# LouisBearing/BirdSoundClassif

Hardware: AMD Instinct MI355X
Metric: clips/sec (3 s @ 22.05 kHz) detect fwd (higher is better)
Workload: dtype f32; 1 GPU; BASELINE.json configs[1]: 1xMI355X inference, batch=64 synthetic 3 s clips (PCM16 @22.05 kHz resident in HBM) through the HIP STFT front end + detector forward + device post-processing, detections returned to the host; batch_per_gpu=64, distinct_clips=64, lanes=2

## Files before the change

birdsoundclassif_amd/_lib.py:

```python
import ctypes as C
import os
import subprocess

_HERE = os.path.dirname(os.path.abspath(__file__))
LIB_PATH = os.environ.get('NBM_LIB') or os.path.join(_HERE, 'libnbm_hip.so')
CSRC = os.path.join(_HERE, 'csrc')

_lib = None


class GemmDesc(C.Structure):
    _fields_ = [('x', C.c_void_p), ('w', C.c_void_p), ('y', C.c_void_p),
                ('scale', C.c_void_p), ('shift', C.c_void_p), ('residual', C.c_void_p),
                ('x_gs', C.c_int64), ('w_gs', C.c_int64), ('y_gs', C.c_int64), ('res_gs', C.c_int64),
                ('groups', C.c_int),
                ('B', C.c_int), ('H', C.c_int), ('W', C.c_int), ('Cin', C.c_int),
                ('N', C.c_int),
                ('kh', C.c_int), ('kw', C.c_int), ('stride', C.c_int), ('pad', C.c_int),
                ('Ho', C.c_int), ('Wo', C.c_int),
                ('x_ld', C.c_int), ('w_ld', C.c_int), ('y_ld', C.c_int), ('res_ld', C.c_int),
                ('alpha', C.c_float), ('act', C.c_int), ('shift_per_row', C.c_int),
                ('up', C.c_void_p), ('up_H', C.c_int), ('up_W', C.c_int),
                ('rows', C.c_void_p), ('rows_blocks', C.c_void_p),
                ('rows_mode', C.c_int), ('rows_count', C.c_int), ('rows_TH', C.c_int), ('rows_TW', C.c_int),
# ... 42 lines not shown
                ('B', C.c_int), ('H', C.c_int), ('W', C.c_int), ('Cin', C.c_int), ('N', C.c_int),
                ('kh', C.c_int), ('kw', C.c_int), ('stride', C.c_int), ('pad', C.c_int), ('Ho', C.c_int), ('Wo', C.c_int),
                ('g_ld', C.c_int), ('w_ld', C.c_int), ('x_ld', C.c_int), ('out_ld', C.c_int), ('res_ld', C.c_int),
                ('mask_ld', C.c_int), ('alpha', C.c_float), ('bias_grad', C.c_void_p), ('residual2', C.c_void_p), ('res2_ld', C.c_int),
                ('mask_bits', C.c_void_p)]


class GemmPlan(C.Structure):
    _fields_ = [('name', C.c_char_p), ('rc', C.c_int), ('kernel', C.c_int), ('grid', C.c_int * 3), ('block', C.c_int),
                ('m_tiles', C.c_int), ('n_tiles', C.c_int), ('vec_epi', C.c_int), ('fast', C.c_int), ('slices', C.c_int),
                ('phased', C.c_int), ('ph_tiles', C.c_int * 4), ('splits', C.c_int), ('k_chunk', C.c_int),
                ('plain', C.c_int), ('b_generic', C.c_int), ('narrow_m', C.c_int), ('halves', C.c_int)]


_P, _I, _L, _F, _U64, _U32 = C.c_void_p, C.c_int, C.c_int64, C.c_float, C.c_uint64, C.c_uint32

SIGNATURES = {
    'nbm_graph_census': [_P, C.POINTER(C.c_longlong * 6)],
    'nbm_copy_rect': [_P, _P, _L, _L, _I, _L, _L, _I, _I, _P],
    'nbm_gemm_conv': [C.POINTER(GemmDesc), _P],
    'nbm_gconv3x3': [C.POINTER(GconvDesc), _P],
    'nbm_gconv3x3_dgrad': [C.POINTER(GconvBwdDesc), _P],
    'nbm_gconv3x3_wgrad': [C.POINTER(GconvBwdDesc), _P],
    'nbm_gconv3x3_wgrad_workspace': [C.POINTER(GconvBwdDesc), C.POINTER(C.c_longlong)],
    'nbm_pcm16_to_wave': [_P, _L, _I, _I, _I, _P, _L, _L, _P, _L, _I, _I, _P],
    'nbm_resample_to_wave': [_P, _L, _I, _L, _I, _I, _P, _I, _L, _L, _P, _L, _I, _I, _I, _P],
    'nbm_wav_decode': [_P, _L, _I, _I, _I, _I, _L, _P, _L, _P],
    'nbm_minmax_init': [_P, _I, _P],
    'nbm_stft_db': [_P, _L, _I, _I, _I, _I, _P, _I, _I, _I, _F, _P, _L, _I, _P, _P],
    'nbm_spec_windows': [_P, _L, _I, _I, _I, _I, _P, _P, _I, _I, _I, _P, _P],
    'nbm_spec_windows_table': [_P, _I, _I, _P, _I, _I, _P],
    'nbm_init_conv': [_P, _L, _P, _P, _I, _P, _P],
    'nbm_stem7x7': [_P, _I, _I, _I, _P, _P, _P, _P, _P, _P, _P],
    'nbm_stem7x7_wgrad': [_P, _P, _I, _I, _I, _P, _P, _P],
    'nbm_maxpool3x3s2': [_P, _I, _I, _I, _I, _P, _I, _I, _P, _P],
    'nbm_space_to_batch2': [_P, _I, _I, _I, _I, _P, _I, _P],
    'nbm_avgpool2x2': [_P, _I, _I, _I, _I, _P, _P],
    'nbm_avgpool2x2_bwd': [_P, _I, _I, _I, _I, _P, _P],
    'nbm_upsample_bilinear_add': [_P, _I, _I, _I, _I, _P, _P, _I, _I, _P],
    'nbm_softmax_rows': [_P, _L, _I, _L, _P],
    'nbm_dwconv3x3': [_P, _I, _I, _I, _I, _I, _I, _P, _P, _P, _L, _P, _I, _I, _P],
    'nbm_dwconv_bn_act': [_P, _I, _I, _I, _I, _I, _I, _P, _P, _P, _I, _P, _I, _I, _P, _P],
    'nbm_dwconv_pool_slots': [_I, _I, _I],
    'nbm_dwconv_strip_rows': [],
    'nbm_se_gate': [_P, _I, _I, _I, _F, _P, _P, _I, _P, _P, _P, _P, _I, _I, _P, _I, _P],
    'nbm_silu': [_P, _P, _L, _P],
    'nbm_layernorm': [_P, _L, _I, _P, _P, _F, _P, _P],
    'nbm_mha_small': [_P, _P, _P, _I, _I, _I, _P, _I, _I, _I, _I, _I, _L, _L, _P, _F, _P],
    'nbm_mha_segments': [_P, _P, _P, _I, _I, _I, _P, _I, _I, _I, _I, _I, _I, _P, _P, _I, _F, _P],
    'nbm_pair_softmax': [_P, _L, _I, _I, _P, _I, _P],
    'nbm_rpn_decode': [_P, _P, _P, _I, _I, _I, _I, _I, _I, _P, _P, _P, _P],
    'nbm_nan_images': [_P, _I, _L, _P, _P],
    'nbm_rpn_select': [_P, _P, _P, _I, _I, _I, _I, _I, _P, _P, _P, _P, _P],
    'nbm_nms_batched': [_P, _P, _P, _I, _I, _F, _I, _P, _P, _P, _P, _P, _P, _P],
    'nbm_rpn_select_big_workspace': [_I, _I, C.POINTER(C.c_int64)],
    'nbm_rpn_select_big': [_P, _P, _P, _I, _I, _I, _I, _I, _P, _L, _P, _P, _P, _P, _P],
    'nbm_nms_big_workspace': [_I, _I, C.POINTER(C.c_int64)],
    'nbm_nms_big': [_P, _P, _P, _I, _I, _F, _I, _P, _L, _P, _P, _P, _P, _P],
    'nbm_roi_pool': [C.POINTER(RoiDesc), _P],
    'nbm_roi_pool_hw': [C.POINTER(RoiHwDesc), _P],
    'nbm_rcnn_post': [_P, _P, _I, _I, _P, _P, _I, _I, _I, _F, _F, _I, _P, _P, _P],
    'nbm_merge_collect': [_P, _P, _I, _I, _I, _I, _I, _L, _P, _P, _P, _P, _P, _P],
    'nbm_merge_nms_workspace': [_I, C.POINTER(C.c_int64)],
    'nbm_merge_nms': [_P, _P, _I, _F, _P, _L, _P, _P, _P],
    'nbm_merge_gather': [_P, _P, _P, _P, _P, _I, _P, _P, _P],
    'nbm_conv_dgrad': [C.POINTER(BwdDesc), _P],
# ... 113 lines not shown
```

birdsoundclassif_amd/csrc/stem.hip:

```cpp
#include "nbm_common.h"

namespace {

constexpr int SP = 264;
constexpr int KR = 8;
constexpr int KK = 7 * KR;
constexpr int OP = 68;
static_assert(7 * SP + KK * 64 <= 128 * OP, "operands must fit the output tile");

struct StemParams {
  const float* img; const float* weff; const float* wb; const float* wb_full; const float* scale; const float* shift;
  float* y;
  int B, H, W, Ho, Wo;
};

__global__ __launch_bounds__(256) void stem7x7_kernel(const StemParams p) {
  __shared__ __attribute__((aligned(16))) float smem[128 * OP];
  float* img_s = smem;
  float* w_s = smem + 7 * SP;
  __shared__ float cb_s[64 * 8];
  const int tid = threadIdx.x, lane = tid & 63, wave = tid >> 6;
  const int ox0 = blockIdx.x * 128, oy = blockIdx.y, b = blockIdx.z;

  const int ix0 = 2 * ox0 - 3;
  constexpr int NST = (7 * SP + 255) / 256;
  float stv[NST];
#pragma unroll
  for (int k = 0; k < NST; ++k) {
    const int i = min(tid + 256 * k, 7 * SP - 1);
    const int r = i / SP, c = i - r * SP;
    const int iy = min(max(2 * oy - 3 + r, 0), p.H - 1), ix = min(max(ix0 + c, 0), p.W - 1);
    stv[k] = p.img[((long long)b * p.H + iy) * p.W + ix];
  }
#pragma unroll
  for (int k = 0; k < NST; ++k) {
    const int i = tid + 256 * k;
    const int r = i / SP, c = i - r * SP;
    const int iy = 2 * oy - 3 + r, ix = ix0 + c;
    if (i < 7 * SP) img_s[i] = ((unsigned)iy < (unsigned)p.H && (unsigned)ix < (unsigned)p.W && c < 261) ? stv[k] : 0.f;
  }
  for (int i = tid; i < KK * 64 / 4; i += 256)
    reinterpret_cast<f32x4*>(w_s)[i] = reinterpret_cast<const f32x4*>(p.weff)[i];
  unsigned rmask = 0;
#pragma unroll
  for (int r = 0; r < 7; ++r)
    if ((unsigned)(2 * oy - 3 + r) < (unsigned)p.H) rmask |= 1u << r;
  const bool row_border = rmask != 0x7fu;
  const bool col_border = ox0 < 2 || 2 * (ox0 + 127) + 3 >= p.W;
  if (row_border || col_border)
    for (int i = tid; i < 64 * 7; i += 256) {
      const int n = i / 7, sx = i - n * 7;
      float a = 0.f;
      for (int r = 0; r < 7; ++r)
        if ((rmask >> r) & 1u) a += p.wb[n * 49 + r * 7 + sx];
      cb_s[n * 8 + sx] = a;
    }
  __syncthreads();

  const int pl = lane & 31, slot = lane >> 5;
  const float* a_base = img_s + 2 * (wave * 32 + pl) + slot;
  const float* b_base = w_s + slot * 64 + pl;
  f32x16 acc0, acc1;
#pragma unroll
  for (int e = 0; e < 16; ++e) { acc0[e] = 0.f; acc1[e] = 0.f; }
#pragma unroll
  for (int j = 0; j < KK / 2; ++j) {
    constexpr int dummy = 0; (void)dummy;
    const int r = (2 * j) / KR, s0 = (2 * j) % KR;
    const float a = a_base[r * SP + s0];
    const float b0 = b_base[(2 * j) * 64], b1 = b_base[(2 * j) * 64 + 32];
    acc0 = __builtin_amdgcn_mfma_f32_32x32x2f32(a, b0, acc0, 0, 0, 0);
    acc1 = __builtin_amdgcn_mfma_f32_32x32x2f32(a, b1, acc1, 0, 0, 0);
  }

  __syncthreads();
#pragma unroll
  for (int t = 0; t < 2; ++t) {
    const int n = 32 * t + pl;
    const float sc = p.scale[n], sh = p.shift[n];
    float bfull = p.wb_full[n];
    if (row_border) {
      bfull = 0.f;
#pragma unroll
      for (int s = 0; s < 7; ++s) bfull += cb_s[n * 8 + s];
    }
    const f32x16& acc = t == 0 ? acc0 : acc1;
#pragma unroll
    for (int e = 0; e < 16; ++e) {
      const int px = wave * 32 + (e & 3) + 8 * (e >> 2) + 4 * slot;
      const int ox = ox0 + px;
      float bias = bfull;
      if (col_border && (ox < 2 || 2 * ox + 3 >= p.W)) {
        bias = 0.f;
#pragma unroll
        for (int s = 0; s < 7; ++s)
          if ((unsigned)(2 * ox - 3 + s) < (unsigned)p.W) bias += cb_s[n * 8 + s];
      }
      smem[px * OP + n] = fmaxf((acc[e] + bias) * sc + sh, 0.f);
    }
  }
  __syncthreads();
  float* yrow = p.y + (((long long)b * p.Ho + oy) * p.Wo + ox0) * 64;
#pragma unroll
  for (int it = 0; it < 8; ++it) {
    const int px = it * 16 + (tid >> 4), c4 = (tid & 15) * 4;
    if (ox0 + px < p.Wo)
      *reinterpret_cast<f32x4*>(yrow + px * 64 + c4) = *reinterpret_cast<const f32x4*>(smem + px * OP + c4);
  }
}

struct StemWgradParams {
  const float* img; const float* g; float* D;
  int B, H, W, Ho, Wo, n_strips, tiles_x;
};

__global__ __launch_bounds__(256) void stem_wgrad_kernel(const StemWgradParams p) {
  __shared__ __attribute__((aligned(16))) float img_s[7 * SP];
  __shared__ __attribute__((aligned(16))) float g_s[128 * 64];
  const int tid = threadIdx.x, lane = tid & 63, wave = tid >> 6;
  const int mt = wave >> 1, nt = wave & 1;
  const int pl = lane & 31, slot = lane >> 5;
  const int col = nt * 32 + pl;
  const int r = col >> 3, sx = col & 7;
  const bool tap = col < 56 && sx < 7;
  const float ones = col == 56 ? 1.f : 0.f;
  const float* b_base = img_s + (tap ? r * SP + sx : 0) + 2 * slot;
  const float* a_base = g_s + slot * 64 + mt * 32 + pl;
  f32x16 acc;
#pragma unroll
  for (int e = 0; e < 16; ++e) acc[e] = 0.f;
  for (int strip = blockIdx.x; strip < p.n_strips; strip += gridDim.x) {
    const int tx = strip % p.tiles_x, rowi = strip / p.tiles_x;
    const int oy = rowi % p.Ho, b = rowi / p.Ho;
    const int ox0 = tx * 128, ix0 = 2 * ox0 - 3;
    __syncthreads();
    constexpr int NST = (7 * SP + 255) / 256;
    float stv[NST];
#pragma unroll
    for (int k = 0; k < NST; ++k) {
      const int i = min(tid + 256 * k, 7 * SP - 1);
// ... 83 lines not shown
extern "C" int nbm_stem7x7_wgrad(const float* img, const float* g, int B, int H, int W, float* D, float* Cb, void* stream) {
  if (!img || !g || !D || !Cb || B <= 0 || H <= 0 || W <= 0) return NBM_EINVAL;
  if (!nbm_aligned16(g)) return NBM_EALIGN;
  StemWgradParams p{};
  p.img = img; p.g = g; p.D = D; p.B = B; p.H = H; p.W = W;
  p.Ho = (H + 6 - 7) / 2 + 1; p.Wo = (W + 6 - 7) / 2 + 1;
  p.tiles_x = (p.Wo + 127) / 128;
  const long long strips = (long long)B * p.Ho * p.tiles_x;
  if (strips > 0x7fffffffll) return NBM_EUNSUPPORTED;
  p.n_strips = (int)strips;
  hipStream_t st = (hipStream_t)stream;
  if (nbm_zero_async(D, sizeof(float) * 64 * 64, st) != hipSuccess || nbm_zero_async(Cb, sizeof(float) * 64 * 49, st) != hipSuccess)
    return (int)hipGetLastError();
  const int grid = (int)(strips < 1024 ? strips : 1024);
  hipLaunchKernelGGL(stem_wgrad_kernel, dim3(grid), dim3(256), 0, st, p);
  int top = p.Ho < 2 ? p.Ho : 2, bot0 = top, left = p.Wo < 2 ? p.Wo : 2, right0 = left;
  while (bot0 < p.Ho && 2 * bot0 + 3 < H) ++bot0;
  while (right0 < p.Wo && 2 * right0 + 3 < W) ++right0;
  hipLaunchKernelGGL(stem_vborder_kernel, dim3(8, B), dim3(256), 0, st, g, H, W, p.Ho, p.Wo, top, bot0, left, right0, Cb);
  return nbm_launch_status();
}

extern "C" int nbm_stem7x7(const float* img, int B, int H, int W, const float* weff, const float* wb, const float* wb_full,
                           const float* scale, const float* shift, float* y, void* stream) {
  if (!img || !weff || !wb || !wb_full || !scale || !shift || !y || B <= 0 || H <= 0 || W <= 0) return NBM_EINVAL;
  if (!nbm_aligned16(weff)) return NBM_EALIGN;
  StemParams p{};
  p.img = img; p.weff = weff; p.wb = wb; p.wb_full = wb_full; p.scale = scale; p.shift = shift; p.y = y;
  p.B = B; p.H = H; p.W = W; p.Ho = (H + 6 - 7) / 2 + 1; p.Wo = (W + 6 - 7) / 2 + 1;
  dim3 grid((p.Wo + 127) / 128, p.Ho, B);
  hipLaunchKernelGGL(stem7x7_kernel, grid, dim3(256), 0, (hipStream_t)stream, p);
  return nbm_launch_status();
}
```

birdsoundclassif_amd/nets/backbone.py:

```python
import math

import torch
from torch import nn

from .. import ops
from . import _prep, functional as Fn
from .position_encoding import build_position_encoding

bcbk_channels = {'resnet': {'2': 64, '3': 256, '4': 512, '5': 1024, '6': 2048}}
_RESNET_LAYERS = {'resnet50': [3, 4, 6, 3], 'resnet101': [3, 4, 23, 3], 'resnet152': [3, 8, 36, 3]}
_RESNEXT = {'resnext50_32x4d': ([3, 4, 6, 3], 32, 4), 'resnext101_32x8d': ([3, 4, 23, 3], 32, 8),
            'resnext101_64x4d': ([3, 4, 23, 3], 64, 4)}
_EFFNET_BASE = ((1, 3, 1, 32, 16, 1), (6, 3, 2, 16, 24, 2), (6, 5, 2, 24, 40, 2), (6, 3, 2, 40, 80, 3), (6, 5, 1, 80, 112, 3),
                (6, 5, 2, 112, 192, 4), (6, 3, 1, 192, 320, 1))
_EFFICIENTNET = {'efficientnet_b0': (1.0, 1.0), 'efficientnet_b1': (1.0, 1.1), 'efficientnet_b2': (1.1, 1.2),
                 'efficientnet_b3': (1.2, 1.4), 'efficientnet_b4': (1.4, 1.8)}
_EFFNET_TAPS = (1, 2, 3, 5, 7)


def _make_divisible(v, divisor=8):
    new_v = max(divisor, int(v + divisor / 2) // divisor * divisor)
    return new_v + divisor if new_v < 0.9 * v else new_v


def efficientnet_stages(name):
    width, depth = _EFFICIENTNET[name]
    return [(t, k, s, _make_divisible(i * width), _make_divisible(o * width), int(math.ceil(n * depth))) for t, k, s, i, o, n in _EFFNET_BASE]


class FrozenBatchNorm2d(nn.Module):

    def __init__(self, n):
        super().__init__()
        self.register_buffer('weight', torch.ones(n))
        self.register_buffer('bias', torch.zeros(n))
        self.register_buffer('running_mean', torch.zeros(n))
        self.register_buffer('running_var', torch.ones(n))

    def _load_from_state_dict(self, state_dict, prefix, local_metadata, strict, missing_keys, unexpected_keys,
                              error_msgs):
        state_dict.pop(prefix + 'num_batches_tracked', None)
        super()._load_from_state_dict(state_dict, prefix, local_metadata, strict, missing_keys, unexpected_keys,
                                      error_msgs)

    def affine(self):
        return _prep.bn_affine(self.weight, self.bias, self.running_mean, self.running_var, 1e-5, frozen=True)


class BatchNorm2d(nn.BatchNorm2d):

# ... 121 lines not shown
            s, b = self.downsample[1].affine()
            idt = Fn.conv(x, self.downsample[0].weight, scale=s, shift=b, stride=self.stride)
        else:
            idt = x
        s, b = self.bn3.affine()
        return Fn.conv(o, self.conv3.weight, scale=s, shift=b, residual=idt, act=ops.ACT_RELU)


class _ResNetBody(nn.Module):

    def __init__(self, layers, norm_layer, dilation=False, groups=1, base_width=64):
        super().__init__()
        self.conv1 = nn.Conv2d(3, 64, 7, stride=2, padding=3, bias=False)
        self.bn1 = norm_layer(64)
        self.dilation = bool(dilation)
        inplanes = 64
        for li, (planes, n, stride) in enumerate(zip((64, 128, 256, 512), layers, (1, 2, 2, 1 if dilation else 2)), start=1):
            blocks = []
            for bi in range(n):
                st = stride if bi == 0 else 1
                ds = None
                if bi == 0 and (st != 1 or inplanes != planes * 4):
                    ds = nn.Sequential(nn.Conv2d(inplanes, planes * 4, 1, stride=st, bias=False), norm_layer(planes * 4))
                blocks.append(_Bottleneck(inplanes, planes, st, ds, norm_layer) if groups == 1 else
                              _GroupedBottleneck(inplanes, planes, st, ds, norm_layer, groups, base_width))
                if dilation and li == 4 and bi > 0:
                    blocks[-1].conv2.dilation, blocks[-1].conv2.padding = (2, 2), (2, 2)
                blocks[-1].mask_input = not (li == 1 and bi == 0)
                blocks[-1].mask_gy = bi == n - 1
                inplanes = planes * 4
            setattr(self, f'layer{li}', nn.Sequential(*blocks))

    def forward(self, x, init_conv=None):
        if _live(self.bn1) and self.training:
            z = Fn.StemRaw.apply(x, init_conv.weight, init_conv.bias, self.conv1.weight) if init_conv is not None else \
                Fn.conv(x, self.conv1.weight, kh=7, kw=7, stride=2, pad=3)
            x = self.bn1.act(z, relu=True)
        else:
            if _live(self.bn1) and torch.is_grad_enabled() and (x.requires_grad or self.conv1.weight.requires_grad or
                                                                self.bn1.weight.requires_grad):
                _refuse_eval_grad('the stem')
            s, b = self.bn1.affine()
            if init_conv is not None:
                x = Fn.Stem.apply(x, init_conv.weight, init_conv.bias, self.conv1.weight, s, b)
            else:
                x = Fn.conv(x, self.conv1.weight, scale=s, shift=b, kh=7, kw=7, stride=2, pad=3, act=ops.ACT_RELU)
        taps = [x]
        x = Fn.MaxPool.apply(x, True)
        for li in range(1, 5):
            for bi, blk in enumerate(getattr(self, f'layer{li}')):
                if self.dilation and li == 4 and bi == 1:
                    x = Fn.SpaceToBatch2.apply(x, False)
                x = blk(x)
            if self.dilation and li == 4 and len(self.layer4) > 1:
                x = Fn.SpaceToBatch2.apply(x, True)
            taps.append(x)
        return taps


class _SqueezeExcitation(nn.Module):

    def __init__(self, channels, squeeze):
        super().__init__()
        self.fc1 = nn.Conv2d(channels, squeeze, 1)
        self.fc2 = nn.Conv2d(squeeze, channels, 1)


def _conv_norm(cin, cout, k, stride, groups, norm_layer):
    return nn.Sequential(nn.Conv2d(cin, cout, k, stride=stride, padding=(k - 1) // 2, groups=groups, bias=False), norm_layer(cout))


class _MBConv(nn.Module):

    def __init__(self, ratio, k, stride, cin, cout, norm_layer):
        super().__init__()
        cexp = _make_divisible(cin * ratio)
        layers = [] if cexp == cin else [_conv_norm(cin, cexp, 1, 1, 1, norm_layer)]
        layers += [_conv_norm(cexp, cexp, k, stride, cexp, norm_layer), _SqueezeExcitation(cexp, max(1, cin // 4)),
                   _conv_norm(cexp, cout, 1, 1, 1, norm_layer)]
        self.block = nn.Sequential(*layers)
        self.k, self.stride, self.use_res = k, stride, stride == 1 and cin == cout
# ... 109 lines not shown
```

birdsoundclassif_amd/nets/functional.py:

```python
import os
import weakref

import torch
from torch.autograd import Function
from torch.autograd.function import once_differentiable

from .. import ops, ondemand
from . import _prep

ACT_NONE, ACT_RELU, ACT_LEAKY = ops.ACT_NONE, ops.ACT_RELU, ops.ACT_LEAKY


def _pad32_rows(g2d, n):
    n32 = (n + 31) // 32 * 32
    if n32 == n:
        return g2d
    out = torch.zeros((g2d.shape[0], n32), device=g2d.device, dtype=torch.float32)
    out[:, :n] = g2d
    return out


GRAD_SINK = {}


# ... 606 lines not shown
    def backward(ctx, g):
        g = g.contiguous()
        gx = ops.dropout(g, *ctx.drop) if ctx.needs_input_grad[0] else None
        return gx, (g if ctx.needs_input_grad[1] else None), None, None, None, None


class Stem(Function):

    @staticmethod
    def forward(ctx, x, w_init, b_init, w1, scale, shift):
        y = ops.stem7x7(x, *_prep.stem_fold(w1, w_init, b_init), scale, shift)
        ctx.save_for_backward(x, w_init, b_init, w1, scale, y)
        return y

    @staticmethod
    @once_differentiable
    def backward(ctx, gy):
        x, w_init, b_init, w1, scale, y = ctx.saved_tensors
        g = gy.contiguous() if _premasked(y, gy) else ops.relu_bwd(gy.contiguous(), y)
        U, V = ops.stem7x7_wgrad(x, g)
        U, V = U * scale.view(64, 1, 1), V * scale.view(64, 1, 1)
        wi, bi = w_init.detach().view(3), b_init.detach().view(3)
        gw1 = wi.view(1, 3, 1, 1) * U[:, None] + bi.view(1, 3, 1, 1) * V[:, None]
        w1d = w1.detach()
        gwi = (w1d * U[:, None]).sum(dim=(0, 2, 3)).view_as(w_init)
        gbi = (w1d * V[:, None]).sum(dim=(0, 2, 3))
        return None, gwi, gbi, gw1, None, None


class MaxPool(Function):

    @staticmethod
    def forward(ctx, x, relu_input=False):
        y, idx = ops.maxpool3x3s2(x, with_index=True)
        ctx.hw = x.shape[1:3]
        ctx.x_ptr, ctx.take_x = x.data_ptr(), stash_accept(x, ctx.needs_input_grad[0])
        ctx.premask = bool(relu_input and ctx.take_x)
        ctx.save_for_backward(idx, x if ctx.premask else None)
        return y

    @staticmethod
    @once_differentiable
    def backward(ctx, gy):
        idx, x = ctx.saved_tensors
        other = _STASH.pop(ctx.x_ptr, None) if ctx.take_x else None
        premask = ctx.premask and other is not None
        gx = ops.maxpool3x3s2_bwd(idx, gy.contiguous(), *ctx.hw, residual=other, mask=x if premask else None)
        ondemand.zero_recycle(other)
        if premask:
            _PREMASKED[ctx.x_ptr] = (gx.data_ptr(), gx._version)
        return gx, None


class SpaceToBatch2(Function):

    @staticmethod
    def forward(ctx, x, inverse):
        ctx.inverse = bool(inverse)
        return ops.space_to_batch2(x, inverse=ctx.inverse)

    @staticmethod
    @once_differentiable
    def backward(ctx, gy):
        return ops.space_to_batch2(gy.contiguous(), inverse=not ctx.inverse), None


class AvgPool2x2(Function):
# ... 421 lines not shown
```

birdsoundclassif_amd/ops.py:

```python
import collections
import ctypes as C
import os
import math

import torch

from . import _lib
from ._lib import GconvBwdDesc, GconvDesc, GemmDesc, RoiHwDesc, check

ACT_NONE, ACT_RELU, ACT_SILU, ACT_LEAKY = 0, 1, 2, 3

PROFILE = None
FLOPS = None
FLOPS_DEFERRED = []


def flops_total():
    tot = FLOPS[0] + sum(float(c.item()) * f for c, f in FLOPS_DEFERRED)
    FLOPS_DEFERRED.clear()
    return tot


_PROFILE_LABEL = None
PROFILE_ONLY = None
# ... 516 lines not shown
    _chk(img, name='img')
    assert tuple(img.shape) == (B, n_bins, w_pix)
    check(lib().nbm_spec_windows_table(_ptr(table), B, n_bins, _ptr(img), w_pix, hop_img, _stream()), 'nbm_spec_windows_table')
    return img


def init_conv(x, w, b):
    _chk(x, name='x')
    C_ = w.numel()
    y = torch.empty(x.shape[:3] + (C_,), device=x.device, dtype=torch.float32)
    check(lib().nbm_init_conv(_ptr(x), x.numel(), _ptr(_chk(w.reshape(-1))), _ptr(_chk(b)), C_, _ptr(y), _stream()),
          'nbm_init_conv')
    return y


def stem7x7(img, weff, wb, wb_full, scale, shift):
    _chk(img, name='img')
    B, H, W = img.shape[:3]
    assert img.numel() == B * H * W and tuple(weff.shape) == (56, 64)
    y = torch.empty((B, (H - 1) // 2 + 1, (W - 1) // 2 + 1, 64), device=img.device, dtype=torch.float32)
    if FLOPS is not None:
        FLOPS[0] += 2.0 * y.numel() * 56
    if _prof_all():
        ev = (torch.cuda.Event(enable_timing=True), torch.cuda.Event(enable_timing=True))
        ev[0].record()
    check(lib().nbm_stem7x7(_ptr(img), B, H, W, _ptr(_chk(weff)), _ptr(_chk(wb)), _ptr(_chk(wb_full)), _ptr(_chk(scale)),
                            _ptr(_chk(shift)), _ptr(y), _stream()), 'nbm_stem7x7')
    if _prof_all():
        ev[1].record()
        PROFILE.append(((1, 64, 7, H, W, B, 1, 2, None), *ev))
    return y


def stem7x7_wgrad(img, g):
    _chk(img, name='img'), _chk(g, name='g')
    B, H, W = img.shape[:3]
    assert g.shape == (B, (H - 1) // 2 + 1, (W - 1) // 2 + 1, 64)
    D = torch.empty((64, 64), device=img.device, dtype=torch.float32)
    Cb = torch.empty((64, 49), device=img.device, dtype=torch.float32)
    check(lib().nbm_stem7x7_wgrad(_ptr(img), _ptr(g), B, H, W, _ptr(D), _ptr(Cb), _stream()), 'nbm_stem7x7_wgrad')
    U = D[:, :56].view(64, 7, 8)[:, :, :7]
    V = D[:, 56].view(64, 1, 1) - Cb.view(64, 7, 7)
    return U, V


def maxpool3x3s2(x, with_index=False):
    _chk(x, name='x')
    B, H, W, C_ = x.shape
    Ho, Wo = (H - 1) // 2 + 1, (W - 1) // 2 + 1
    y = torch.empty((B, Ho, Wo, C_), device=x.device, dtype=torch.float32)
    idx = torch.empty((B, Ho, Wo, C_), device=x.device, dtype=torch.uint8) if with_index else None
    check(lib().nbm_maxpool3x3s2(_ptr(x), B, H, W, C_, _ptr(y), Ho, Wo, _ptr(idx), _stream()), 'nbm_maxpool3x3s2')
    return (y, idx) if with_index else y


def space_to_batch2(x, inverse=False):
    _chk(x, name='x')
    if inverse:
        B4, h, w, C_ = x.shape
        assert B4 % 4 == 0
        B, H, W = B4 // 4, 2 * h, 2 * w
        y = torch.empty((B, H, W, C_), device=x.device, dtype=torch.float32)
    else:
        B, H, W, C_ = x.shape
        if (H | W) & 1:
            raise NotImplementedError('space_to_batch2 needs even map sizes (the dilated ResNet stage at 24 x 64)')
# ... 1050 lines not shown
```

include/nbm_hip.h:

```cpp
#ifndef NBM_HIP_H
#define NBM_HIP_H

#include <stdint.h>

#ifdef __cplusplus
extern "C" {
#endif

#define NBM_OK 0
#define NBM_EINVAL (-1)
#define NBM_EALIGN (-2)
#define NBM_EUNSUPPORTED (-3)

#define NBM_ACT_NONE 0
#define NBM_ACT_RELU 1
#define NBM_ACT_SILU 2
#define NBM_ACT_LEAKY 3

const char* nbm_version(void);

int nbm_graph_census(void* graph, long long counts[6]);

typedef struct nbm_gemm_desc {
  const float* x;
// ... 115 lines not shown

int nbm_resample_to_wave(const float* x, int64_t x_ld, int batch, int64_t n, int L, int M, const double* taps, int T,
                         int64_t first, int64_t count, float* out, int64_t out_ld, int lead, int pad_mode, int quant16,
                         void* stream);

#define NBM_WAV_MAX_CHANNELS 8
int nbm_wav_decode(const void* raw, int64_t raw_pitch, int batch, int tag, int bits, int channels, int64_t n, float* out,
                   int64_t out_pitch, void* stream);

int nbm_minmax_init(uint32_t* minmax, int batch, void* stream);
int nbm_stft_db(const float* wave, int64_t wave_ld, int batch, int n_frames, int hop, int n_fft,
                const double* basis, int basis_bin_tiles, int basis_ksteps, int n_bins, float floor_amp,
                float* db, int64_t db_bs, int db_ld, uint32_t* minmax, void* stream);

int nbm_spec_windows(const float* db, int64_t db_bs, int db_ld, int batch, int n_bins, int n_frames,
                     const uint32_t* minmax, float* img, int n_img, int w_pix, int hop_img,
                     const int32_t* last_cols, void* stream);

typedef struct nbm_window_entry {
  const float* db;
  const uint32_t* minmax;
  const int32_t* last_cols;
  int32_t db_ld, n_frames, window, n_img;
} nbm_window_entry;

int nbm_spec_windows_table(const nbm_window_entry* table, int batch, int n_bins, float* img, int w_pix, int hop_img,
                           void* stream);


int nbm_init_conv(const float* x, int64_t n_pix, const float* w, const float* b, int C, float* y, void* stream);

int nbm_stem7x7(const float* img, int B, int H, int W, const float* weff, const float* wb, const float* wb_full,
                const float* scale, const float* shift, float* y, void* stream);

int nbm_stem7x7_wgrad(const float* img, const float* g, int B, int H, int W, float* D, float* Cb, void* stream);

int nbm_maxpool3x3s2(const float* x, int B, int H, int W, int C, float* y, int Ho, int Wo, uint8_t* idx, void* stream);
int nbm_space_to_batch2(const float* x, int B, int H, int W, int C, float* y, int inverse, void* stream);
int nbm_avgpool2x2(const float* x, int B, int Ho, int Wo, int C, float* y, void* stream);
int nbm_avgpool2x2_bwd(const float* gy, int B, int Ho, int Wo, int C, float* gx, void* stream);

int nbm_upsample_bilinear_add(const float* src, int B, int Hi, int Wi, int C, const float* add,
                              float* y, int Ho, int Wo, void* stream);

int nbm_softmax_rows(float* x, int64_t rows, int cols, int64_t ld, void* stream);

int nbm_dwconv3x3(const float* x, int B, int H, int W, int Cin, int mult, int stride,
                  const float* w , const float* bias, const float* film, int64_t film_ld,
                  float* y, int Ho, int Wo, void* stream);

int nbm_dwconv_bn_act(const float* x, int B, int H, int W, int C, int k, int stride, const float* w_taps, const float* scale,
                      const float* shift, int act, float* y, int Ho, int Wo, float* pool_part, void* stream);
int nbm_dwconv_pool_slots(int C, int Ho, int Wo);
int nbm_dwconv_strip_rows(void);
int nbm_se_gate(const float* pool_part, int B, int n_slots, int C, float inv_hw, const float* w1, const float* b1, int Csq,
                const float* w2, const float* b2, float* gate, const float* wproj, int wp_ld, int N, float* wb, int w_ld, void* stream);

int nbm_silu(const float* x, float* y, int64_t n, void* stream);

int nbm_layernorm(const float* x, int64_t rows, int E, const float* w, const float* b, float eps, float* y, void* stream);

int nbm_mha_small(const float* q, const float* k, const float* v, int q_ld, int k_ld, int v_ld, float* out, int out_ld,
                  int S, int N, int nhead, int hd, int64_t seq_stride, int64_t batch_stride, const int32_t* n_valid,
                  float scale, void* stream);

#define NBM_MHA_ACROSS_ROIS 0
// ... 231 lines not shown
```

Measured before the change: 1087 clips/s.

## Fuse stem 7x7 conv with 3x3/s2 maxpool behind env flag; skip pool index

Adds a stem kernel that computes three conv output rows per pooled row, sweeps column tiles with software-prefetched input staging, and writes both the stem output and the max-pooled output, exchanging tile-edge values through shared memory. This is meant to remove the separate maxpool launch and its reread of the stem activation. The fused path is gated by NBM_STEM_POOL, which defaults to off, and is taken only in no-grad inference. Separately, MaxPool skips writing the argmax index when no input gradient is needed, which does run by default in inference.

```diff
diff --git a/birdsoundclassif_amd/_lib.py b/birdsoundclassif_amd/_lib.py
--- a/birdsoundclassif_amd/_lib.py
+++ b/birdsoundclassif_amd/_lib.py
@@ -98,6 +98,7 @@
     'nbm_spec_windows_table': [_P, _I, _I, _P, _I, _I, _P],
     'nbm_init_conv': [_P, _L, _P, _P, _I, _P, _P],
     'nbm_stem7x7': [_P, _I, _I, _I, _P, _P, _P, _P, _P, _P, _P],
+    'nbm_stem7x7_pool': [_P, _I, _I, _I, _P, _P, _P, _P, _P, _P, _P, _P],
     'nbm_stem7x7_wgrad': [_P, _P, _I, _I, _I, _P, _P, _P],
     'nbm_maxpool3x3s2': [_P, _I, _I, _I, _I, _P, _I, _I, _P, _P],
     'nbm_space_to_batch2': [_P, _I, _I, _I, _I, _P, _I, _P],
diff --git a/birdsoundclassif_amd/csrc/stem.hip b/birdsoundclassif_amd/csrc/stem.hip
--- a/birdsoundclassif_amd/csrc/stem.hip
+++ b/birdsoundclassif_amd/csrc/stem.hip
@@ -13,6 +13,112 @@
   float* y;
   int B, H, W, Ho, Wo;
 };
+
+template <int NR>
+constexpr int stem_nst() { return (NR * SP + 255) / 256; }
+
+template <int NR>
+__device__ __forceinline__ void stem_stage_load(const StemParams& p, int b, int iy0, int ix0, int tid, float (&stv)[stem_nst<NR>()]) {
+#pragma unroll
+  for (int k = 0; k < stem_nst<NR>(); ++k) {
+    const int i = min(tid + 256 * k, NR * SP - 1);
+    const int r = i / SP, c = i - r * SP;
+    const int iy = min(max(iy0 + r, 0), p.H - 1), ix = min(max(ix0 + c, 0), p.W - 1);
+    stv[k] = p.img[((long long)b * p.H + iy) * p.W + ix];
+  }
+}
+
+template <int NR>
+__device__ __forceinline__ void stem_stage_write(const StemParams& p, int iy0, int ix0, int tid, const float (&stv)[stem_nst<NR>()],
+                                                 float* img_s) {
+#pragma unroll
+  for (int k = 0; k < stem_nst<NR>(); ++k) {
+    const int i = tid + 256 * k;
+    const int r = i / SP, c = i - r * SP;
+    const int iy = iy0 + r, ix = ix0 + c;
+    if (i < NR * SP) img_s[i] = ((unsigned)iy < (unsigned)p.H && (unsigned)ix < (unsigned)p.W && c < 261) ? stv[k] : 0.f;
+  }
+}
+
+__device__ __forceinline__ unsigned stem_rmask(int oy, int H) {
+  unsigned rmask = 0;
+#pragma unroll
+  for (int r = 0; r < 7; ++r)
+    if ((unsigned)(2 * oy - 3 + r) < (unsigned)H) rmask |= 1u << r;
+  return rmask;
+}
+
+__device__ __forceinline__ void stem_cb_rows(const float* wb, unsigned rmask, int tid, float* cb) {
+  for (int i = tid; i < 64 * 7; i += 256) {
+    const int n = i / 7, sx = i - n * 7;
+    float v[7], a = 0.f;
+#pragma unroll
+    for (int r = 0; r < 7; ++r) v[r] = wb[n * 49 + r * 7 + sx];
+#pragma unroll
+    for (int r = 0; r < 7; ++r)
+      if ((rmask >> r) & 1u) a += v[r];
+    cb[n * 8 + sx] = a;
+  }
+}
+
+__device__ __forceinline__ void stem_mfma(const float* a_base, const float* b_base, f32x16& acc0, f32x16& acc1) {
+#pragma unroll
+  for (int e = 0; e < 16; ++e) { acc0[e] = 0.f; acc1[e] = 0.f; }
+#pragma unroll
+  for (int j = 0; j < KK / 2; ++j) {
+    const int r = (2 * j) / KR, s0 = (2 * j) % KR;
+    const float a = a_base[r * SP + s0];
+    const float b0 = b_base[(2 * j) * 64], b1 = b_base[(2 * j) * 64 + 32];
+    acc0 = __builtin_amdgcn_mfma_f32_32x32x2f32(a, b0, acc0, 0, 0, 0);
+    acc1 = __builtin_amdgcn_mfma_f32_32x32x2f32(a, b1, acc1, 0, 0, 0);
+  }
+}
+
+struct StemAffine { float sc[2], sh[2], bfull[2]; };
+
+__device__ __forceinline__ StemAffine stem_affine(const StemParams& p, int pl) {
+  StemAffine af;
+#pragma unroll
+  for (int t = 0; t < 2; ++t) { af.sc[t] = p.scale[32 * t + pl]; af.sh[t] = p.shift[32 * t + pl]; af.bfull[t] = p.wb_full[32 * t + pl]; }
+  return af;
+}
+
+template <class Put>
+__device__ __forceinline__ void stem_epilogue(const StemParams& p, const StemAffine& af, const float* cb, bool row_border,
+                                              bool col_border, int ox0, int wave, int pl, int slot, const f32x16& acc0,
+                                              const f32x16& acc1, Put&& put) {
+#pragma unroll
+  for (int t = 0; t < 2; ++t) {
+    const int n = 32 * t + pl;
+    const float sc = af.sc[t], sh = af.sh[t];
+    float bfull = af.bfull[t];
+    if (row_border) {
+      bfull = 0.f;
+#pragma unroll
+      for (int s = 0; s < 7; ++s) bfull += cb[n * 8 + s];
+    }
+    const f32x16& acc = t == 0 ? acc0 : acc1;
+    float bias[16];
+#pragma unroll
+    for (int e = 0; e < 16; ++e) bias[e] = bfull;
+    if (col_border) {
+#pragma unroll
+      for (int e = 0; e < 16; ++e) {
+        const int ox = ox0 + wave * 32 + (e & 3) + 8 * (e >> 2) + 4 * slot;
+        if (ox < 2 || 2 * ox + 3 >= p.W) {
+          float bs = 0.f;
+#pragma unroll
+          for (int s = 0; s < 7; ++s)
+            if ((unsigned)(2 * ox - 3 + s) < (unsigned)p.W) bs += cb[n * 8 + s];
+          bias[e] = bs;
+        }
+      }
+    }
+#pragma unroll
+    for (int e = 0; e < 16; ++e)
+      put(t, e, wave * 32 + (e & 3) + 8 * (e >> 2) + 4 * slot, n, fmaxf((acc[e] + bias[e]) * sc + sh, 0.f));
+  }
+}
 
 __global__ __launch_bounds__(256) void stem7x7_kernel(const StemParams p) {
   __shared__ __attribute__((aligned(16))) float smem[128 * OP];
@@ -20,85 +126,28 @@
   float* w_s = smem + 7 * SP;
   __shared__ float cb_s[64 * 8];
   const int tid = threadIdx.x, lane = tid & 63, wave = tid >> 6;
+  const int pl = lane & 31, slot = lane >> 5;
   const int ox0 = blockIdx.x * 128, oy = blockIdx.y, b = blockIdx.z;
+  const StemAffine af = stem_affine(p, pl);
 
   const int ix0 = 2 * ox0 - 3;
-  constexpr int NST = (7 * SP + 255) / 256;
-  float stv[NST];
-#pragma unroll
-  for (int k = 0; k < NST; ++k) {
-    const int i = min(tid + 256 * k, 7 * SP - 1);
-    const int r = i / SP, c = i - r * SP;
-    const int iy = min(max(2 * oy - 3 + r, 0), p.H - 1), ix = min(max(ix0 + c, 0), p.W - 1);
-    stv[k] = p.img[((long long)b * p.H + iy) * p.W + ix];
-  }
-#pragma unroll
-  for (int k = 0; k < NST; ++k) {
-    const int i = tid + 256 * k;
-    const int r = i / SP, c = i - r * SP;
-    const int iy = 2 * oy - 3 + r, ix = ix0 + c;
-    if (i < 7 * SP) img_s[i] = ((unsigned)iy < (unsigned)p.H && (unsigned)ix < (unsigned)p.W && c < 261) ? stv[k] : 0.f;
-  }
+  float stv[stem_nst<7>()];
+  stem_stage_load<7>(p, b, 2 * oy - 3, ix0, tid, stv);
+  stem_stage_write<7>(p, 2 * oy - 3, ix0, tid, stv, img_s);
   for (int i = tid; i < KK * 64 / 4; i += 256)
     reinterpret_cast<f32x4*>(w_s)[i] = reinterpret_cast<const f32x4*>(p.weff)[i];
-  unsigned rmask = 0;
-#pragma unroll
-  for (int r = 0; r < 7; ++r)
-    if ((unsigned)(2 * oy - 3 + r) < (unsigned)p.H) rmask |= 1u << r;
+  const unsigned rmask = stem_rmask(oy, p.H);
   const bool row_border = rmask != 0x7fu;
   const bool col_border = ox0 < 2 || 2 * (ox0 + 127) + 3 >= p.W;
-  if (row_border || col_border)
-    for (int i = tid; i < 64 * 7; i += 256) {
-      const int n = i / 7, sx = i - n * 7;
-      float a = 0.f;
-      for (int r = 0; r < 7; ++r)
-        if ((rmask >> r) & 1u) a += p.wb[n * 49 + r * 7 + sx];
-      cb_s[n * 8 + sx] = a;
-    }
+  if (row_border || col_border) stem_cb_rows(p.wb, rmask, tid, cb_s);
   __syncthreads();
 
-  const int pl = lane & 31, slot = lane >> 5;
-  const float* a_base = img_s + 2 * (wave * 32 + pl) + slot;
-  const float* b_base = w_s + slot * 64 + pl;
   f32x16 acc0, acc1;
-#pragma unroll
-  for (int e = 0; e < 16; ++e) { acc0[e] = 0.f; acc1[e] = 0.f; }
-#pragma unroll
-  for (int j = 0; j < KK / 2; ++j) {
-    constexpr int dummy = 0; (void)dummy;
-    const int r = (2 * j) / KR, s0 = (2 * j) % KR;
-    const float a = a_base[r * SP + s0];
-    const float b0 = b_base[(2 * j) * 64], b1 = b_base[(2 * j) * 64 + 32];
-    acc0 = __builtin_amdgcn_mfma_f32_32x32x2f32(a, b0, acc0, 0, 0, 0);
-    acc1 = __builtin_amdgcn_mfma_f32_32x32x2f32(a, b1, acc1, 0, 0, 0);
-  }
+  stem_mfma(img_s + 2 * (wave * 32 + pl) + slot, w_s + slot * 64 + pl, acc0, acc1);
 
   __syncthreads();
-#pragma unroll
-  for (int t = 0; t < 2; ++t) {
-    const int n = 32 * t + pl;
-    const float sc = p.scale[n], sh = p.shift[n];
-    float bfull = p.wb_full[n];
-    if (row_border) {
-      bfull = 0.f;
-#pragma unroll
-      for (int s = 0; s < 7; ++s) bfull += cb_s[n * 8 + s];
-    }
-    const f32x16& acc = t == 0 ? acc0 : acc1;
-#pragma unroll
-    for (int e = 0; e < 16; ++e) {
-      const int px = wave * 32 + (e & 3) + 8 * (e >> 2) + 4 * slot;
-      const int ox = ox0 + px;
-      float bias = bfull;
-      if (col_border && (ox < 2 || 2 * ox + 3 >= p.W)) {
-        bias = 0.f;
-#pragma unroll
-        for (int s = 0; s < 7; ++s)
-          if ((unsigned)(2 * ox - 3 + s) < (unsigned)p.W) bias += cb_s[n * 8 + s];
-      }
-      smem[px * OP + n] = fmaxf((acc[e] + bias) * sc + sh, 0.f);
-    }
-  }
+  stem_epilogue(p, af, cb_s, row_border, col_border, ox0, wave, pl, slot, acc0, acc1,
+                [&](int, int, int px, int n, float v) { smem[px * OP + n] = v; });
   __syncthreads();
   float* yrow = p.y + (((long long)b * p.Ho + oy) * p.Wo + ox0) * 64;
 #pragma unroll
@@ -106,6 +155,99 @@
     const int px = it * 16 + (tid >> 4), c4 = (tid & 15) * 4;
     if (ox0 + px < p.Wo)
       *reinterpret_cast<f32x4*>(yrow + px * 64 + c4) = *reinterpret_cast<const f32x4*>(smem + px * OP + c4);
+  }
+}
+
+constexpr int PR = 11;
+
+struct StemPoolParams {
+  StemParams s;
+  float* yp;
+  int Hp, Wp;
+};
+
+__global__ __launch_bounds__(256, 2) void stem7x7_pool_kernel(const StemPoolParams q) {
+  __shared__ __attribute__((aligned(16))) float w_s[KK * 64];
+  __shared__ __attribute__((aligned(16))) float img_s[PR * SP];
+  __shared__ float cb_s[3 * 64 * 8];
+  __shared__ float edge_s[5 * 64];
+  const StemParams& p = q.s;
+  const int tid = threadIdx.x, lane = tid & 63, wave = tid >> 6;
+  const int pl = lane & 31, slot = lane >> 5;
+  const int py = blockIdx.x, b = blockIdx.y;
+  const int iy0 = 4 * py - 5;
+  const int ntx = (p.Wo + 127) / 128;
+
+  const StemAffine af = stem_affine(p, pl);
+  float stv[stem_nst<PR>()];
+  stem_stage_load<PR>(p, b, iy0, -3, tid, stv);
+  for (int i = tid; i < KK * 64 / 4; i += 256)
+    reinterpret_cast<f32x4*>(w_s)[i] = reinterpret_cast<const f32x4*>(p.weff)[i];
+  for (int rr = 0; rr < 3; ++rr) stem_cb_rows(p.wb, stem_rmask(2 * py - 1 + rr, p.H), tid, cb_s + rr * 512);
+  stem_stage_write<PR>(p, iy0, -3, tid, stv, img_s);
+  __syncthreads();
+
+  const float* a_base = img_s + 2 * (wave * 32 + pl) + slot;
+  const float* b_base = w_s + slot * 64 + pl;
+  for (int tx = 0; tx < ntx; ++tx) {
+    const int ox0 = tx * 128;
+    const bool more = tx + 1 < ntx;
+    if (more) stem_stage_load<PR>(p, b, iy0, 2 * (ox0 + 128) - 3, tid, stv);
+    const bool col_border = ox0 < 2 || 2 * (ox0 + 127) + 3 >= p.W;
+    float vm[2][16];
+#pragma unroll
+    for (int e = 0; e < 16; ++e) vm[0][e] = vm[1][e] = -INFINITY;
+#pragma unroll 1
+    for (int k = 0; k < 3; ++k) {
+      const int rr = k == 2 ? 0 : k + 1;
+      const int oy = 2 * py - 1 + rr;
+      if ((unsigned)oy >= (unsigned)p.Ho) continue;
+      f32x16 acc0, acc1;
+      stem_mfma(a_base + 2 * rr * SP, b_base, acc0, acc1);
+      float* ylane = p.y + (((long long)b * p.Ho + oy) * p.Wo + ox0 + wave * 32 + 4 * slot) * 64 + pl;
+      int ox0k = ox0;
+      asm volatile("" : "+s"(ox0k));
+      const float* cb = cb_s + rr * 512;
+      const bool row_border = stem_rmask(oy, p.H) != 0x7fu;
+      auto offset = [](int t, int e) { return ((e & 3) + 8 * (e >> 2)) * 64 + 32 * t; };
+      if (rr == 0)
+        stem_epilogue(p, af, cb, row_border, col_border, ox0k, wave, pl, slot, acc0, acc1,
+                      [&](int t, int e, int, int, float v) { vm[t][e] = fmaxf(vm[t][e], v); });
+      else if (ox0k + 128 <= p.Wo)
+        stem_epilogue(p, af, cb, row_border, col_border, ox0k, wave, pl, slot, acc0, acc1, [&](int t, int e, int, int, float v) {
+          vm[t][e] = fmaxf(vm[t][e], v);
+          ylane[offset(t, e)] = v;
+        });
+      else
+        stem_epilogue(p, af, cb, row_border, col_border, ox0k, wave, pl, slot, acc0, acc1, [&](int t, int e, int px, int, float v) {
+          vm[t][e] = fmaxf(vm[t][e], v);
+          if (ox0k + px < p.Wo) ylane[offset(t, e)] = v;
+        });
+    }
+    float* edge_out = edge_s + (wave < 3 ? wave : 3 + (tx & 1)) * 64;
+    if (slot == 1) { edge_out[pl] = vm[0][15]; edge_out[32 + pl] = vm[1][15]; }
+    __syncthreads();
+    if (more) stem_stage_write<PR>(p, iy0, 2 * (ox0 + 128) - 3, tid, stv, img_s);
+    const float* edge_in = edge_s + (wave > 0 ? wave - 1 : 3 + ((tx & 1) ^ 1)) * 64;
+    float* plane = q.yp + (((long long)b * q.Hp + py) * q.Wp + ox0 / 2 + wave * 16 + 2 * slot) * 64 + pl;
+#pragma unroll
+    for (int t = 0; t < 2; ++t) {
+      const int n = 32 * t + pl;
+#pragma unroll
+      for (int g = 0; g < 4; ++g) {
+        const float mine = slot == 0 ? vm[t][4 * g + 3] : vm[t][g > 0 ? 4 * g - 1 : 0];
+        float left = __shfl_xor(mine, 32);
+        if (g == 0 && slot == 0) left = edge_in[n];
+        const int c = wave * 32 + 8 * g + 4 * slot, ox = ox0 + c;
+        float m0 = fmaxf(vm[t][4 * g], -INFINITY), m1 = fmaxf(vm[t][4 * g + 2], -INFINITY);
+        if (ox > 0) m0 = fmaxf(m0, left);
+        if (ox + 1 < p.Wo) { m0 = fmaxf(m0, vm[t][4 * g + 1]); m1 = fmaxf(m1, vm[t][4 * g + 1]); }
+        if (ox + 3 < p.Wo) m1 = fmaxf(m1, vm[t][4 * g + 3]);
+        if (ox / 2 < q.Wp) plane[(4 * g) * 64 + 32 * t] = m0;
+        if (ox / 2 + 1 < q.Wp) plane[(4 * g + 1) * 64 + 32 * t] = m1;
+      }
+    }
+    __syncthreads();
   }
 }
 
@@ -255,3 +397,17 @@
   hipLaunchKernelGGL(stem7x7_kernel, grid, dim3(256), 0, (hipStream_t)stream, p);
   return nbm_launch_status();
 }
+
+extern "C" int nbm_stem7x7_pool(const float* img, int B, int H, int W, const float* weff, const float* wb, const float* wb_full,
+                                const float* scale, const float* shift, float* y, float* yp, void* stream) {
+  if (!img || !weff || !wb || !wb_full || !scale || !shift || !y || !yp || B <= 0 || H <= 0 || W <= 0) return NBM_EINVAL;
+  if (!nbm_aligned16(weff) || !nbm_aligned16(y) || !nbm_aligned16(yp)) return NBM_EALIGN;
+  if (B > 65535) return NBM_EUNSUPPORTED;
+  StemPoolParams q{};
+  StemParams& p = q.s;
+  p.img = img; p.weff = weff; p.wb = wb; p.wb_full = wb_full; p.scale = scale; p.shift = shift; p.y = y;
+  p.B = B; p.H = H; p.W = W; p.Ho = (H + 6 - 7) / 2 + 1; p.Wo = (W + 6 - 7) / 2 + 1;
+  q.yp = yp; q.Hp = (p.Ho - 1) / 2 + 1; q.Wp = (p.Wo - 1) / 2 + 1;
+  hipLaunchKernelGGL(stem7x7_pool_kernel, dim3(q.Hp, B), dim3(256), 0, (hipStream_t)stream, q);
+  return nbm_launch_status();
+}
diff --git a/birdsoundclassif_amd/nets/backbone.py b/birdsoundclassif_amd/nets/backbone.py
--- a/birdsoundclassif_amd/nets/backbone.py
+++ b/birdsoundclassif_amd/nets/backbone.py
@@ -1,4 +1,5 @@
 import math
+import os
 
 import torch
 from torch import nn
@@ -16,6 +17,7 @@
 _EFFICIENTNET = {'efficientnet_b0': (1.0, 1.0), 'efficientnet_b1': (1.0, 1.1), 'efficientnet_b2': (1.1, 1.2),
                  'efficientnet_b3': (1.2, 1.4), 'efficientnet_b4': (1.4, 1.8)}
 _EFFNET_TAPS = (1, 2, 3, 5, 7)
+STEM_POOL = os.environ.get('NBM_STEM_POOL', '0') == '1'
 
 
 def _make_divisible(v, divisor=8):
@@ -203,6 +205,7 @@
             setattr(self, f'layer{li}', nn.Sequential(*blocks))
 
     def forward(self, x, init_conv=None):
+        pooled = None
         if _live(self.bn1) and self.training:
             z = Fn.StemRaw.apply(x, init_conv.weight, init_conv.bias, self.conv1.weight) if init_conv is not None else \
                 Fn.conv(x, self.conv1.weight, kh=7, kw=7, stride=2, pad=3)
@@ -212,12 +215,14 @@
                                                                 self.bn1.weight.requires_grad):
                 _refuse_eval_grad('the stem')
             s, b = self.bn1.affine()
-            if init_conv is not None:
+            if init_conv is not None and STEM_POOL and not torch.is_grad_enabled():
+                x, pooled = ops.stem7x7_pool(x, *_prep.stem_fold(self.conv1.weight, init_conv.weight, init_conv.bias), s, b)
+            elif init_conv is not None:
                 x = Fn.Stem.apply(x, init_conv.weight, init_conv.bias, self.conv1.weight, s, b)
             else:
                 x = Fn.conv(x, self.conv1.weight, scale=s, shift=b, kh=7, kw=7, stride=2, pad=3, act=ops.ACT_RELU)
         taps = [x]
-        x = Fn.MaxPool.apply(x, True)
+        x = Fn.MaxPool.apply(x, True) if pooled is None else pooled
         for li in range(1, 5):
             for bi, blk in enumerate(getattr(self, f'layer{li}')):
                 if self.dilation and li == 4 and bi == 1:
diff --git a/birdsoundclassif_amd/nets/functional.py b/birdsoundclassif_amd/nets/functional.py
--- a/birdsoundclassif_amd/nets/functional.py
+++ b/birdsoundclassif_amd/nets/functional.py
@@ -662,7 +662,10 @@
 
     @staticmethod
     def forward(ctx, x, relu_input=False):
-        y, idx = ops.maxpool3x3s2(x, with_index=True)
+        if ctx.needs_input_grad[0]:
+            y, idx = ops.maxpool3x3s2(x, with_index=True)
+        else:
+            y, idx = ops.maxpool3x3s2(x), None
         ctx.hw = x.shape[1:3]
         ctx.x_ptr, ctx.take_x = x.data_ptr(), stash_accept(x, ctx.needs_input_grad[0])
         ctx.premask = bool(relu_input and ctx.take_x)
diff --git a/birdsoundclassif_amd/ops.py b/birdsoundclassif_amd/ops.py
--- a/birdsoundclassif_amd/ops.py
+++ b/birdsoundclassif_amd/ops.py
@@ -572,6 +572,26 @@
     return y
 
 
+def stem7x7_pool(img, weff, wb, wb_full, scale, shift):
+    _chk(img, name='img')
+    B, H, W = img.shape[:3]
+    assert img.numel() == B * H * W and tuple(weff.shape) == (56, 64)
+    Ho, Wo = (H - 1) // 2 + 1, (W - 1) // 2 + 1
+    y = torch.empty((B, Ho, Wo, 64), device=img.device, dtype=torch.float32)
+    yp = torch.empty((B, (Ho - 1) // 2 + 1, (Wo - 1) // 2 + 1, 64), device=img.device, dtype=torch.float32)
+    if FLOPS is not None:
+        FLOPS[0] += 2.0 * y.numel() * 56
+    if _prof_all():
+        ev = (torch.cuda.Event(enable_timing=True), torch.cuda.Event(enable_timing=True))
+        ev[0].record()
+    check(lib().nbm_stem7x7_pool(_ptr(img), B, H, W, _ptr(_chk(weff)), _ptr(_chk(wb)), _ptr(_chk(wb_full)), _ptr(_chk(scale)),
+                                 _ptr(_chk(shift)), _ptr(y), _ptr(yp), _stream()), 'nbm_stem7x7_pool')
+    if _prof_all():
+        ev[1].record()
+        PROFILE.append(((1, 64, 7, H, W, B, 1, 2, None), *ev))
+    return y, yp
+
+
 def stem7x7_wgrad(img, g):
     _chk(img, name='img'), _chk(g, name='g')
     B, H, W = img.shape[:3]
diff --git a/include/nbm_hip.h b/include/nbm_hip.h
--- a/include/nbm_hip.h
+++ b/include/nbm_hip.h
@@ -171,6 +171,9 @@
 
 int nbm_stem7x7(const float* img, int B, int H, int W, const float* weff, const float* wb, const float* wb_full,
                 const float* scale, const float* shift, float* y, void* stream);
+
+int nbm_stem7x7_pool(const float* img, int B, int H, int W, const float* weff, const float* wb, const float* wb_full,
+                     const float* scale, const float* shift, float* y, float* yp, void* stream);
 
 int nbm_stem7x7_wgrad(const float* img, const float* g, int B, int H, int W, float* D, float* Cb, void* stream);
 
```

Result: no change. 1090 clips/s, median of 2 (+0.3%).
